# aapdo/M3ViT

Hardware: AMD Instinct MI355X
Metric: images/sec fwd+bwd ViT-S/16 MoE(E=16,k=4) 224^2 bs=128 (higher is better)
Workload: dtype f16; 1 GPU; configs[1]: ViT-Small/16 + MoE E=16 top-k=4 multi_gate, synthetic 224x224; batch_per_gpu=128, global_batch=128, task_passes=2, launch=hipGraph replay (one linear graph per task pass and stream), routing=deterministic (std=0), task_streams=2, wgrad_streams=0, activation_checkpointing=False, parallelism=single, full=False

## Files before the change

### m3vit_amd/csrc/gemm.hip

```cpp
#include <stdlib.h>
#include "gemm_dev.h"

using namespace m3;

struct GemmEnv {
  int band;
  bool dma;
  bool tall;
};
static int env_int(const char *name, int unset) { const char *e = getenv(name); return e ? atoi(e) : unset; }
static const GemmEnv &gemm_env() {
  static const GemmEnv env = {env_int("M3_GEMM_BAND", 0), env_int("M3_GEMM_DMA", 1) != 0, env_int("M3_GEMM_F32_TALL", 1) != 0};
  return env;
}

static int g_big_mode = -1;
extern "C" int m3_gemm_set_big(int mode) {
  M3_REQUIRE(mode >= -1 && mode <= 2, "m3_gemm_set_big: mode %d out of range", mode);
  g_big_mode = mode;
  return M3_OK;
}

static int epilogue_kind(const m3_gemm_args *a) {
  if (dtype_size(a->dtype) != 2) return DMA_EPI_ANY;
  const bool c_f32 = a->c_dtype == M3_F32, none = a->act == M3_ACT_NONE && !a->pre_out;
  if (none && a->gelu_grad_pre && !a->residual && !c_f32 && !a->bias) return DMA_EPI_GPRE;
  if (none && a->residual && !a->gelu_grad_pre && c_f32) return DMA_EPI_RES;
  if (none && !a->gelu_grad_pre && !a->residual && !c_f32) return DMA_EPI_PLAIN;
  if (a->act == M3_ACT_GELU && a->pre_out && !a->gelu_grad_pre && !a->residual && !c_f32) return DMA_EPI_GELU;
  return DMA_EPI_ANY;
}

enum GemmKernel { GEMM_BIG, GEMM_DMA, GEMM_STAGED, GEMM_STAGED_TALL };

static GemmKernel choose_kernel(const GemmDev &d, int dtype) {
  const GemmEnv &env = gemm_env();
  const int es = dtype_size(dtype);
  if (g_big_mode < 0) g_big_mode = env_int("M3_GEMM_BIG", 2);
  if (g_big_mode && gemm_big_eligible(d, es, g_big_mode == 1)) return GEMM_BIG;
  if (env.dma && es == 2 && d.vec8 && (d.K * es) % ROWB == 0) return GEMM_DMA;
  if (env.tall && dtype == M3_F32 && (d.K * es) % ROWB == 0 && !d.group_offsets) {
    const int64_t nt = (d.N + BN - 1) / BN, t128 = (d.M + 127) / 128 * nt, t160 = (d.M + 159) / 160 * nt;
    if ((t160 + 255) / 256 * 160 < (t128 + 255) / 256 * 128) return GEMM_STAGED_TALL;
  }
  return GEMM_STAGED;
}

struct GemmLaunch { GemmDev d; GemmKernel kernel; int epi, tile_m, tile_n; bool empty; };
static int gemm_prepare(const m3_gemm_args *a, const char *who, GemmLaunch &L) {
  M3_REQUIRE(a && a->A && a->B && a->C, "%s: null operand", who);
  M3_REQUIRE(dtype_ok(a->dtype), "%s: bad dtype %d", who, a->dtype);
  const int es = dtype_size(a->dtype);
  M3_REQUIRE(a->M >= 0 && a->N > 0 && a->K > 0, "%s: bad shape M=%lld N=%d K=%d", who, (long long)a->M, a->N, a->K);
  M3_REQUIRE((a->K * es) % 16 == 0, "%s: K*elem (%d) must be a multiple of 16 bytes", who, a->K * es);
  M3_REQUIRE((a->lda * es) % 16 == 0 && (a->ldb * es) % 16 == 0, "%s: lda/ldb rows must be 16-byte aligned", who);
  M3_REQUIRE(((uintptr_t)a->A % 16) == 0 && ((uintptr_t)a->B % 16) == 0 && ((uintptr_t)a->C % 16) == 0,
             "%s: operands must be 16-byte aligned", who);
  M3_REQUIRE(a->N % 4 == 0 && a->ldc % 4 == 0, "%s: N and ldc must be multiples of 4", who);
  M3_REQUIRE(a->lda >= a->K && a->ldb >= a->K && a->ldc >= a->N, "%s: leading dimension too small", who);
  M3_REQUIRE(a->c_dtype == M3_F32 || a->c_dtype == a->dtype, "%s: c_dtype must be f32 or the operand dtype", who);
  M3_REQUIRE(a->G >= 1, "%s: G must be >= 1", who);
  M3_REQUIRE((a->group_offsets == nullptr) == (a->tile_starts == nullptr), "%s: group_offsets/tile_starts go together", who);
  M3_REQUIRE(a->G == 1 || a->group_offsets, "%s: grouped call needs group_offsets", who);
  M3_REQUIRE(!a->a_row_idx || a->a_row_div >= 1, "%s: a_row_div must be >= 1", who);
  M3_REQUIRE(!a->pre_out || a->ld_pre % 4 == 0, "%s: ld_pre %% 4", who);
  M3_REQUIRE(!a->gelu_grad_pre || a->ld_gpre % 4 == 0, "%s: ld_gpre %% 4", who);
  M3_REQUIRE(!a->residual || a->ld_res % 4 == 0, "%s: ld_res %% 4", who);
  M3_REQUIRE(!a->row_scale || a->row_scale_div >= 1, "%s: row_scale_div must be >= 1", who);
  L.empty = a->M == 0;
  if (L.empty) return M3_OK;

  GemmDev &d = L.d;
  d.A = (const char *)a->A; d.lda_b = a->lda * es;
  d.a_row_idx = a->a_row_idx; d.a_row_div = a->a_row_idx ? a->a_row_div : 1;
  d.a_row_sh = div_shift(d.a_row_div);
  d.B = (const char *)a->B; d.ldb_b = a->ldb * es; d.b_group_b = (int64_t)a->N * a->ldb * es;
  d.C = (char *)a->C; d.ldc = a->ldc; d.c_f32 = (a->c_dtype == M3_F32) ? 1 : 0;
  d.c_row_idx = a->c_row_idx;
  d.bias = a->bias;
  d.pre_out = (char *)a->pre_out; d.ld_pre = a->ld_pre;
  d.gpre = (const char *)a->gelu_grad_pre; d.ld_gpre = a->ld_gpre;
  d.residual = a->residual; d.ld_res = a->ld_res;
  d.row_scale = a->row_scale; d.row_scale_div = a->row_scale ? a->row_scale_div : 1;
  d.row_scale_idx = a->row_scale ? a->row_scale_idx : nullptr;
  d.act = a->act;
  d.M = a->M; d.N = a->N; d.K = a->K; d.G = a->G;
  d.group_offsets = a->group_offsets; d.tile_starts = a->tile_starts;
  d.a_seg_tiles = 0; d.a_seg_jump_b = 0;
  d.vec8 = (a->N % 8 == 0 && a->ldc % 8 == 0 && (!a->pre_out || a->ld_pre % 8 == 0) &&
            (!a->gelu_grad_pre || a->ld_gpre % 8 == 0) && (!a->residual || a->ld_res % 8 == 0)) ? 1 : 0;
  M3_REQUIRE((a->M + 1) * a->lda * es < ((int64_t)1 << 32) && (int64_t)a->N * a->ldb * es < ((int64_t)1 << 32),
             "%s: operand panel exceeds the 4 GiB reach of the 32-bit lane offsets", who);

  const GemmKernel kernel = L.kernel = choose_kernel(d, a->dtype);
  L.epi = kernel == GEMM_BIG || kernel == GEMM_DMA ? epilogue_kind(a) : DMA_EPI_ANY;
  const int tile_m = L.tile_m = kernel == GEMM_BIG ? BIG_B : kernel == GEMM_STAGED_TALL ? 160 : BM;
  const int tile_n = L.tile_n = kernel == GEMM_BIG ? BIG_B : BN;
  const int band = gemm_env().band > 0 ? gemm_env().band : ((int64_t)a->N * a->K * es > ((int64_t)2 << 20) ? 4 : 1);
  const int64_t mt = (a->M + tile_m - 1) / tile_m + (a->group_offsets ? a->G : 0);
  d.n_tiles = (a->N + tile_n - 1) / tile_n;
  d.m_band = kernel == GEMM_BIG ? 1 : band;
  M3_REQUIRE(mt * d.n_tiles < (int64_t)1 << 30, "%s: grid too large", who);
  d.m_tiles_max = (int)mt;
  return M3_OK;
}

extern "C" int m3_gemm_nt(const m3_gemm_args *a, void *stream) {
  GemmLaunch L;
  if (int rc = gemm_prepare(a, "m3_gemm_nt", L)) return rc;
  if (L.empty) return M3_OK;
  hipStream_t s = (hipStream_t)stream;
  switch (L.kernel) {
    case GEMM_BIG: return launch_gemm_big(L.d, a->dtype, L.epi, s);
    case GEMM_DMA: return launch_gemm_dma(L.d, a->dtype, L.epi, s);
    default: return launch_gemm_staged(L.d, a->dtype, L.kernel == GEMM_STAGED_TALL, s);
  }
}

extern "C" int m3_gemm_plan(const m3_gemm_args *a, m3_gemm_plan_out *p) {
  M3_REQUIRE(p, "m3_gemm_plan: null output");
  GemmLaunch L;
  if (int rc = gemm_prepare(a, "m3_gemm_plan", L)) return rc;
  *p = m3_gemm_plan_out{};
  p->kernel = M3_GEMM_NONE;
  if (L.empty) return M3_OK;
  p->kernel = L.kernel == GEMM_BIG ? M3_GEMM_BIG : L.kernel == GEMM_DMA ? M3_GEMM_DMA : L.kernel == GEMM_STAGED_TALL ? M3_GEMM_STAGED_TALL : M3_GEMM_STAGED;
  p->epilogue = L.epi; p->tile_m = L.tile_m; p->tile_n = L.tile_n; p->m_band = L.d.m_band; p->vec8 = L.d.vec8;
  p->n_tiles = L.d.n_tiles; p->m_tiles_max = L.d.m_tiles_max;
  return M3_OK;
}
```

### m3vit_amd/csrc/gemm_dev.h

```cpp
#pragma once
#include <type_traits>
#include "common.h"

namespace m3 {

constexpr int BM = 128, BN = 128, ROWB = 128;
constexpr int GEMM_THREADS = 256;

struct GemmDev {
  const char *A; int64_t lda_b;
  const int32_t *a_row_idx; int32_t a_row_div; int32_t a_row_sh;
  const char *B; int64_t ldb_b; int64_t b_group_b;
  char *C; int64_t ldc; int32_t c_f32;
  const int32_t *c_row_idx;
  const float *bias;
  char *pre_out; int64_t ld_pre;
  const char *gpre; int64_t ld_gpre;
  const float *residual; int64_t ld_res;
  const float *row_scale; int32_t row_scale_div;
  const int32_t *row_scale_idx;
  int32_t act;
  int64_t M; int32_t N; int32_t K;
  int32_t G;
  const int32_t *group_offsets;
  const int32_t *tile_starts;
  int32_t n_tiles;
  int32_t m_band;
  int32_t m_tiles_max;
  int32_t vec8;
  int32_t a_seg_tiles; int64_t a_seg_jump_b;
};

struct TileOwner { int g; int64_t m_begin, m_end; };
__device__ __forceinline__ int grouped_live_tiles(const int32_t *tile_starts, int G, int lane, int &ts_lane) {
  if (G <= 64) {
    ts_lane = lane < G ? tile_starts[lane + 1] : 0x7fffffff;
    return __builtin_amdgcn_readfirstlane(__shfl(ts_lane, G - 1, 64));
  }
  ts_lane = 0;
  return tile_starts[G];
}
template <int ROWS>
__device__ __forceinline__ TileOwner grouped_tile_rows(const int32_t *group_offsets, int g, int t0, int mt) {
  TileOwner o;
  g = __builtin_amdgcn_readfirstlane(g);
  t0 = __builtin_amdgcn_readfirstlane(t0);
  o.g = g;
  o.m_begin = (int64_t)__builtin_amdgcn_readfirstlane(group_offsets[g]) + (int64_t)(mt - t0) * ROWS;
  o.m_end = __builtin_amdgcn_readfirstlane(group_offsets[g + 1]);
  return o;
}
__device__ __forceinline__ TileOwner grouped_tile_owner(const int32_t *tile_starts, const int32_t *group_offsets, int G,
                                                        int mt, int lane, int ts_lane) {
  int g = 0, t0;
  if (G <= 64) {
    g = __popcll(__ballot(lane < G - 1 && ts_lane <= mt));
    t0 = g ? __shfl(ts_lane, g - 1, 64) : 0;
  } else {
    while (g + 1 < G && tile_starts[g + 1] <= mt) ++g;
    t0 = tile_starts[g];
  }
  return grouped_tile_rows<128>(group_offsets, g, t0, mt);
}

__device__ __forceinline__ int dma_swz(int row) { return (row >> 1) & 7; }

enum { DMA_EPI_ANY = 0, DMA_EPI_GPRE = 1, DMA_EPI_RES = 2, DMA_EPI_PLAIN = 3, DMA_EPI_GELU = 4 };

template <typename F> inline void with_epi(int epi, F &&f) {
  switch (epi) {
    case DMA_EPI_GPRE: f(std::integral_constant<int, DMA_EPI_GPRE>()); break;
    case DMA_EPI_RES: f(std::integral_constant<int, DMA_EPI_RES>()); break;
    case DMA_EPI_PLAIN: f(std::integral_constant<int, DMA_EPI_PLAIN>()); break;
    case DMA_EPI_GELU: f(std::integral_constant<int, DMA_EPI_GELU>()); break;
    default: f(std::integral_constant<int, DMA_EPI_ANY>()); break;
  }
}

template <typename T, typename RowFactor>
__device__ __forceinline__ void epilogue_row_any(const GemmDev &p, int64_t m, int n, f32x4 v0, f32x4 v1, RowFactor row_factor) {
  const int64_t crow = p.c_row_idx ? (int64_t)p.c_row_idx[m] : m;
  if (p.pre_out) Vec8<T>::store((T *)p.pre_out + crow * p.ld_pre + n, v0, v1);
  if (p.act == M3_ACT_GELU) {
#pragma unroll
    for (int j = 0; j < 4; ++j) { v0[j] = gelu_f(v0[j]); v1[j] = gelu_f(v1[j]); }
  }
  if (p.gpre) {
    f32x4 p0, p1;
    Vec8<T>::load((const T *)p.gpre + crow * p.ld_gpre + n, p0, p1);
#pragma unroll
    for (int j = 0; j < 4; ++j) { v0[j] *= gelu_grad_f(p0[j]); v1[j] *= gelu_grad_f(p1[j]); }
  }
  if (p.row_scale) {
    const float sc = row_factor(crow);
    v0 *= sc; v1 *= sc;
  }
  if (p.residual) {
    v0 += *(const f32x4 *)(p.residual + crow * p.ld_res + n);
    v1 += *(const f32x4 *)(p.residual + crow * p.ld_res + n + 4);
  }
  if (p.c_f32) {
    *(f32x4 *)((float *)p.C + crow * p.ldc + n) = v0;
    *(f32x4 *)((float *)p.C + crow * p.ldc + n + 4) = v1;
  } else {
    Vec8<T>::store((T *)p.C + crow * p.ldc + n, v0, v1);
  }
}

constexpr int BIG_B = 256;
int launch_gemm_staged(const GemmDev &d, int dtype, bool tall, hipStream_t s);
int launch_gemm_dma(const GemmDev &d, int dtype, int epi, hipStream_t s);
bool gemm_big_eligible(const GemmDev &d, int dtype_size_bytes, bool force);
int launch_gemm_big(const GemmDev &d, int dtype, int epi, hipStream_t s);
int launch_gemm_big_seg(const GemmDev &d, int dtype, hipStream_t s, const char *who);

__device__ __forceinline__ void tile_of(int t, int n_tiles, int m_band, int live_m, int &mt, int &nt) {
  if (m_band <= 1) { mt = t / n_tiles; nt = t - mt * n_tiles; return; }
  const int per = m_band * n_tiles;
  const int band = t / per, r = t - band * per;
  const int rows = min(m_band, live_m - band * m_band);
  nt = r / rows;
  mt = band * m_band + (r - nt * rows);
}
}
```

### m3vit_amd/csrc/gemm_dma.hip

```cpp
#include "gemm_dev.h"

namespace m3 {

constexpr int DMA_RB = 128;
constexpr int DMA_LDS = 2 * BM * DMA_RB;
constexpr int DMA_LDS_ALL = DMA_LDS + BM * 4;

template <typename T, int EPI, bool HINT>
__global__ __launch_bounds__(GEMM_THREADS, 4) void gemm_nt_dma_kernel(const GemmDev p) {
  typedef Mma<T> MM;
  typedef typename MM::frag frag;
  constexpr int RB = DMA_RB;
  constexpr int OPB = BM * RB;
  constexpr int CPR = RB / 16;
  constexpr int RPI = 64 / CPR;
  constexpr int NPC = BM / RPI / 4;
  constexpr int KCH = RB / 64;
  extern __shared__ __attribute__((aligned(16))) char smem[];

  const int tid = threadIdx.x;
  const int lane = tid & 63, wave = __builtin_amdgcn_readfirstlane(tid >> 6);
  const int li = lane & 15, lg = lane >> 4;
  const int wr = wave >> 1, wc = wave & 1;

  int ts_lane = 0;
  const int nwg = p.tile_starts ? grouped_live_tiles(p.tile_starts, p.G, lane, ts_lane) * p.n_tiles : (int)gridDim.x;
  if ((int)blockIdx.x >= nwg) return;
  const int t = xcd_remap(blockIdx.x, nwg);
  int mt, nt;
  tile_of(t, p.n_tiles, p.m_band, nwg / p.n_tiles, mt, nt);
  int g = 0;
  int64_t m_begin, m_end;
  if (p.tile_starts) {
    const TileOwner ow = grouped_tile_owner(p.tile_starts, p.group_offsets, p.G, mt, lane, ts_lane);
    g = ow.g; m_begin = ow.m_begin; m_end = ow.m_end;
  } else {
    m_begin = (int64_t)mt * BM;
    m_end = p.M;
    if (m_begin >= m_end) return;
  }
  const int n0 = nt * BN;

  const char *a_src[NPC], *b_src[NPC];
  int64_t mrow[NPC];
  int32_t aix[NPC];
#pragma unroll
  for (int j = 0; j < NPC; ++j) {
    const int row = (NPC * wave + j) * RPI + lane / CPR;
    int64_t m = m_begin + row;
    if (m >= m_end) m = m_end - 1;
    mrow[j] = m;
  }
  if (p.a_row_idx) {
#pragma unroll
    for (int j = 0; j < NPC; ++j) aix[j] = p.a_row_idx[mrow[j]];
  }
  const bool want_rs = p.row_scale && tid < BM;
  const int32_t *rs_idx = p.row_scale_idx ? p.row_scale_idx : p.c_row_idx;
  int64_t rs_m = m_begin + tid;
  if (rs_m >= m_end) rs_m = m_end - 1;
  int32_t rs_ix = 0;
  if (want_rs && rs_idx) rs_ix = rs_idx[rs_m];
  float my_rs = 1.0f;
  if (want_rs) {
    const int64_t srow = rs_idx ? (int64_t)rs_ix : rs_m;
    my_rs = p.row_scale[p.row_scale_div == 1 ? srow : srow / p.row_scale_div];
  }
#pragma unroll
  for (int j = 0; j < NPC; ++j) {
    const int row = (NPC * wave + j) * RPI + lane / CPR;
    const int c = (lane % CPR) ^ dma_swz(row);
    const int64_t src = p.a_row_idx ? (int64_t)div_by(aix[j], p.a_row_div, p.a_row_sh) : mrow[j];
    a_src[j] = p.A + src * p.lda_b + c * 16;
    int n = n0 + row;
    if (n >= p.N) n = p.N - 1;
    b_src[j] = p.B + (int64_t)g * p.b_group_b + (int64_t)n * p.ldb_b + c * 16;
  }
  const int nk = (p.K * (int)sizeof(T)) / RB;

  typedef __attribute__((address_space(3))) void lds_void;
  typedef const __attribute__((address_space(1))) void glb_void;
  auto dma = [&](int ks) {
    char *dst = smem + (NPC * wave) * 1024;
#pragma unroll
    for (int j = 0; j < NPC; ++j) {
      __builtin_amdgcn_global_load_lds((glb_void *)(a_src[j] + ks * RB), (lds_void *)(dst + j * 1024), 16, 0, 0);
      __builtin_amdgcn_global_load_lds((glb_void *)(b_src[j] + ks * RB), (lds_void *)(dst + j * 1024 + OPB), 16, 0, 0);
    }
  };

  int rdA[KCH], rdB[KCH];
#pragma unroll
  for (int kc = 0; kc < KCH; ++kc) {
    rdA[kc] = (wr * 64 + li) * RB + (((kc * 4 + lg) ^ dma_swz(li)) << 4);
    rdB[kc] = (wc * 64 + li) * RB + (((kc * 4 + lg) ^ dma_swz(li)) << 4) + OPB;
  }

  f32x4 acc[4][4];
#pragma unroll
  for (int a = 0; a < 4; ++a)
#pragma unroll
    for (int b = 0; b < 4; ++b) acc[a][b] = f32x4{0.f, 0.f, 0.f, 0.f};

  auto compute = [&]() {
    const char *sb = smem;
#pragma unroll
    for (int kc = 0; kc < KCH; ++kc) {
      frag fa[4], fb[4];
#pragma unroll
      for (int i = 0; i < 4; ++i) {
        fa[i] = *(const frag *)(sb + rdA[kc] + i * 16 * RB);
        fb[i] = *(const frag *)(sb + rdB[kc] + i * 16 * RB);
      }
#pragma unroll
      for (int ni = 0; ni < 4; ++ni)
#pragma unroll
        for (int mi = 0; mi < 4; ++mi) acc[ni][mi] = MM::mma(fb[ni], fa[mi], acc[ni][mi]);
    }
  };

  for (int ks = 0; ks < nk; ++ks) {
    dma(ks);
    __syncthreads();
    compute();
    __syncthreads();
  }

  const float *bias = p.bias ? p.bias + (int64_t)g * p.N : nullptr;
  const int cg = tid & 15, r16 = tid >> 4;
  const int n = n0 + cg * 8;
  f32x4 b0 = f32x4{0.f, 0.f, 0.f, 0.f}, b1 = b0;
  if (bias && n < p.N) { b0 = *(const f32x4 *)(bias + n); b1 = *(const f32x4 *)(bias + n + 4); }
  float *const s_rs = (float *)(smem + DMA_LDS);
  if (tid < BM) s_rs[tid] = my_rs;
#pragma unroll
  for (int h = 0; h < 2; ++h) {
    u32x4 gq[4];
    f32x4 rq[4][2];
    int32_t crow4[4];
    constexpr int NPRE = EPI == DMA_EPI_RES ? 2 : 4;
    auto fetch_epi = [&](int ps) {
      if constexpr (EPI == DMA_EPI_GPRE) gq[ps] = ld_nt<HINT>((const u32x4 *)((const T *)p.gpre + (int64_t)crow4[ps] * p.ld_gpre + n));
      if constexpr (EPI == DMA_EPI_RES) {
        rq[ps][0] = *(const f32x4 *)(p.residual + (int64_t)crow4[ps] * p.ld_res + n);
        rq[ps][1] = *(const f32x4 *)(p.residual + (int64_t)crow4[ps] * p.ld_res + n + 4);
      }
    };
    if constexpr (EPI != DMA_EPI_ANY) {
      if (n < p.N) {
#pragma unroll
        for (int ps = 0; ps < 4; ++ps) {
          int64_t m = m_begin + h * 64 + ps * 16 + r16;
          if (m >= m_end) m = m_end - 1;
          crow4[ps] = p.c_row_idx ? p.c_row_idx[m] : (int32_t)m;
        }
#pragma unroll
        for (int ps = 0; ps < NPRE; ++ps) fetch_epi(ps);
      }
    }
    if (h) __syncthreads();
    if (wr == h) {
#pragma unroll
      for (int mi = 0; mi < 4; ++mi)
#pragma unroll
        for (int ni = 0; ni < 4; ++ni) {
          const int lrow = mi * 16 + li;
          const int chunk = wc * 16 + ni * 4 + lg;
          *(f32x4 *)(smem + lrow * 512 + ((chunk ^ (lrow & 31)) << 4)) = acc[ni][mi];
        }
    }
    __syncthreads();
    if constexpr (EPI != DMA_EPI_ANY) {
      if (n < p.N) {
#pragma unroll
        for (int ps = NPRE; ps < 4; ++ps) fetch_epi(ps);
#pragma unroll
        for (int ps = 0; ps < 4; ++ps) {
          const int lrow = ps * 16 + r16;
          const int64_t crow = crow4[ps];
          const int sw = lrow & 31;
          f32x4 v0 = *(const f32x4 *)(smem + lrow * 512 + (((2 * cg) ^ sw) << 4));
          f32x4 v1 = *(const f32x4 *)(smem + lrow * 512 + (((2 * cg + 1) ^ sw) << 4));
          v0 += b0; v1 += b1;
          if constexpr (EPI == DMA_EPI_GELU) {
            if constexpr (HINT) st_nt<true>((u32x4 *)((T *)p.pre_out + crow * p.ld_pre + n), pack8<T>(v0, v1));
            else Vec8<T>::store((T *)p.pre_out + crow * p.ld_pre + n, v0, v1);
#pragma unroll
            for (int j = 0; j < 4; ++j) { v0[j] = gelu_f(v0[j]); v1[j] = gelu_f(v1[j]); }
          }
          if constexpr (EPI == DMA_EPI_GPRE) {
            typedef T t8 __attribute__((ext_vector_type(8)));
            const t8 pr = __builtin_bit_cast(t8, gq[ps]);
#pragma unroll
            for (int j = 0; j < 4; ++j) { v0[j] *= gelu_grad_f((float)pr[j]); v1[j] *= gelu_grad_f((float)pr[4 + j]); }
          }
          const float sc = s_rs[h * 64 + lrow];
          v0 *= sc; v1 *= sc;
          if constexpr (EPI == DMA_EPI_RES) {
            v0 += rq[ps][0]; v1 += rq[ps][1];
            if (m_begin + h * 64 + lrow < m_end) {
              *(f32x4 *)((float *)p.C + crow * p.ldc + n) = v0;
              *(f32x4 *)((float *)p.C + crow * p.ldc + n + 4) = v1;
            }
          } else {
            Vec8<T>::store((T *)p.C + crow * p.ldc + n, v0, v1);
          }
        }
      }
    } else if (n < p.N) {
#pragma unroll 2
      for (int ps = 0; ps < 4; ++ps) {
        const int lrow = ps * 16 + r16;
        const int64_t m = m_begin + h * 64 + lrow;
        if (m >= m_end) break;
        const int sw = lrow & 31;
        const f32x4 v0 = *(const f32x4 *)(smem + lrow * 512 + (((2 * cg) ^ sw) << 4));
        const f32x4 v1 = *(const f32x4 *)(smem + lrow * 512 + (((2 * cg + 1) ^ sw) << 4));
        epilogue_row_any<T>(p, m, n, v0 + b0, v1 + b1, [&](int64_t) { return s_rs[h * 64 + lrow]; });
      }
    }
  }
}

int launch_gemm_dma(const GemmDev &d, int dtype, int epi, hipStream_t s) {
  const dim3 grid((unsigned)((int64_t)d.m_tiles_max * d.n_tiles)), block(GEMM_THREADS);
  const int hints = cache_hints();
  auto go = [&](auto t) {
    with_epi(epi, [&](auto e) {
      constexpr int EPI = decltype(e)::value;
      constexpr int BIT = EPI == DMA_EPI_GELU ? M3_HINT_GEMM_PRE : EPI == DMA_EPI_GPRE ? M3_HINT_GEMM_GPRE : 0;
      if (BIT && (hints & BIT)) {
        hipLaunchKernelGGL((gemm_nt_dma_kernel<decltype(t), EPI, BIT != 0>), grid, block, DMA_LDS_ALL, s, d);
      } else {
        hipLaunchKernelGGL((gemm_nt_dma_kernel<decltype(t), EPI, false>), grid, block, DMA_LDS_ALL, s, d);
      }
    });
  };
  if (dtype == M3_F16) go(half_t());
  else go(bf16_t());
  return check_launch("m3_gemm_nt");
}

}
```

Before: 8002 images/s.

## Shrink DMA GEMM prologue: scalar params, 32-bit offsets, hoisted first load

The DMA GEMM kernel now copies its parameters into values pinned to scalar registers. It replaces 64-bit per-piece source pointers with 32-bit lane offsets from a scalar base, and computes tile row bounds in 32-bit arithmetic with a precomputed shift for row-scale division. The first K-slice DMA is issued before the loop, and each later slice is issued after the compute barrier. This shortens the prologue and cuts VGPR pressure. A new host check limits M to 32 bits, and optional timestamp instrumentation is added behind a compile flag.

```diff
diff --git a/m3vit_amd/csrc/gemm.hip b/m3vit_amd/csrc/gemm.hip
--- a/m3vit_amd/csrc/gemm.hip
+++ b/m3vit_amd/csrc/gemm.hip
@@ -83,6 +83,7 @@
   d.residual = a->residual; d.ld_res = a->ld_res;
   d.row_scale = a->row_scale; d.row_scale_div = a->row_scale ? a->row_scale_div : 1;
   d.row_scale_idx = a->row_scale ? a->row_scale_idx : nullptr;
+  d.row_scale_sh = div_shift(d.row_scale_div);
   d.act = a->act;
   d.M = a->M; d.N = a->N; d.K = a->K; d.G = a->G;
   d.group_offsets = a->group_offsets; d.tile_starts = a->tile_starts;
@@ -91,6 +92,7 @@
             (!a->gelu_grad_pre || a->ld_gpre % 8 == 0) && (!a->residual || a->ld_res % 8 == 0)) ? 1 : 0;
   M3_REQUIRE((a->M + 1) * a->lda * es < ((int64_t)1 << 32) && (int64_t)a->N * a->ldb * es < ((int64_t)1 << 32),
              "%s: operand panel exceeds the 4 GiB reach of the 32-bit lane offsets", who);
+  M3_REQUIRE(a->M < ((int64_t)1 << 31), "%s: M %lld does not fit 32 bits", who, (long long)a->M);
 
   const GemmKernel kernel = L.kernel = choose_kernel(d, a->dtype);
   L.epi = kernel == GEMM_BIG || kernel == GEMM_DMA ? epilogue_kind(a) : DMA_EPI_ANY;
diff --git a/m3vit_amd/csrc/gemm_dev.h b/m3vit_amd/csrc/gemm_dev.h
--- a/m3vit_amd/csrc/gemm_dev.h
+++ b/m3vit_amd/csrc/gemm_dev.h
@@ -19,6 +19,7 @@
   const float *residual; int64_t ld_res;
   const float *row_scale; int32_t row_scale_div;
   const int32_t *row_scale_idx;
+  int32_t row_scale_sh;
   int32_t act;
   int64_t M; int32_t N; int32_t K;
   int32_t G;
@@ -50,9 +51,9 @@
   o.m_end = __builtin_amdgcn_readfirstlane(group_offsets[g + 1]);
   return o;
 }
-__device__ __forceinline__ TileOwner grouped_tile_owner(const int32_t *tile_starts, const int32_t *group_offsets, int G,
-                                                        int mt, int lane, int ts_lane) {
-  int g = 0, t0;
+__device__ __forceinline__ void grouped_tile_group(const int32_t *tile_starts, int G, int mt, int lane, int ts_lane, int &g,
+                                                   int &t0) {
+  g = 0;
   if (G <= 64) {
     g = __popcll(__ballot(lane < G - 1 && ts_lane <= mt));
     t0 = g ? __shfl(ts_lane, g - 1, 64) : 0;
@@ -60,6 +61,11 @@
     while (g + 1 < G && tile_starts[g + 1] <= mt) ++g;
     t0 = tile_starts[g];
   }
+}
+__device__ __forceinline__ TileOwner grouped_tile_owner(const int32_t *tile_starts, const int32_t *group_offsets, int G,
+                                                        int mt, int lane, int ts_lane) {
+  int g, t0;
+  grouped_tile_group(tile_starts, G, mt, lane, ts_lane, g, t0);
   return grouped_tile_rows<128>(group_offsets, g, t0, mt);
 }
 
diff --git a/m3vit_amd/csrc/gemm_dma.hip b/m3vit_amd/csrc/gemm_dma.hip
--- a/m3vit_amd/csrc/gemm_dma.hip
+++ b/m3vit_amd/csrc/gemm_dma.hip
@@ -5,6 +5,17 @@
 constexpr int DMA_RB = 128;
 constexpr int DMA_LDS = 2 * BM * DMA_RB;
 constexpr int DMA_LDS_ALL = DMA_LDS + BM * 4;
+
+#ifdef M3_GEMM_STAMPS
+constexpr int STAMP_WGS = 4096, STAMP_N = 64;
+__device__ unsigned long long g_gemm_stamps[STAMP_WGS][STAMP_N];
+#define M3_GEMM_STAMP(i)                                                                                              \
+  do {                                                                                                                \
+    if (threadIdx.x == 0 && blockIdx.x < STAMP_WGS && (i) < STAMP_N) g_gemm_stamps[blockIdx.x][(i)] = __builtin_amdgcn_s_memtime(); \
+  } while (0)
+#else
+#define M3_GEMM_STAMP(i) do { } while (0)
+#endif
 
 template <typename T, int EPI, bool HINT>
 __global__ __launch_bounds__(GEMM_THREADS, 4) void gemm_nt_dma_kernel(const GemmDev p) {
@@ -18,76 +29,120 @@
   constexpr int KCH = RB / 64;
   extern __shared__ __attribute__((aligned(16))) char smem[];
 
+  M3_GEMM_STAMP(0);
+  const char *const A = p.A, *const B = p.B;
+  const int64_t lda_b = p.lda_b, ldb_b = p.ldb_b, b_group_b = p.b_group_b, M = p.M;
+  const int32_t *const a_row_idx = p.a_row_idx, *const c_row_idx = p.c_row_idx, *const row_scale_idx = p.row_scale_idx;
+  const int32_t *const group_offsets = p.group_offsets, *const tile_starts = p.tile_starts;
+  const float *const row_scale = p.row_scale;
+  const int a_row_div = p.a_row_div, a_row_sh = p.a_row_sh, row_scale_div = p.row_scale_div, row_scale_sh = p.row_scale_sh;
+  const int N = p.N, K = p.K, G = p.G, n_tiles = p.n_tiles, m_band = p.m_band, m_tiles_max = p.m_tiles_max;
+  asm volatile("" ::"s"(A), "s"(B), "s"(lda_b), "s"(ldb_b), "s"(b_group_b), "s"(M), "s"(a_row_idx), "s"(c_row_idx),
+               "s"(row_scale_idx), "s"(group_offsets), "s"(tile_starts), "s"(row_scale), "s"(a_row_div), "s"(a_row_sh),
+               "s"(row_scale_div), "s"(row_scale_sh), "s"(N), "s"(K), "s"(G), "s"(n_tiles), "s"(m_band), "s"(m_tiles_max));
+
   const int tid = threadIdx.x;
   const int lane = tid & 63, wave = __builtin_amdgcn_readfirstlane(tid >> 6);
   const int li = lane & 15, lg = lane >> 4;
   const int wr = wave >> 1, wc = wave & 1;
 
   int ts_lane = 0;
-  const int nwg = p.tile_starts ? grouped_live_tiles(p.tile_starts, p.G, lane, ts_lane) * p.n_tiles : (int)gridDim.x;
+  const int live_m = tile_starts ? grouped_live_tiles(tile_starts, G, lane, ts_lane) : m_tiles_max;
+  const int nwg = live_m * n_tiles;
   if ((int)blockIdx.x >= nwg) return;
   const int t = xcd_remap(blockIdx.x, nwg);
   int mt, nt;
-  tile_of(t, p.n_tiles, p.m_band, nwg / p.n_tiles, mt, nt);
-  int g = 0;
-  int64_t m_begin, m_end;
-  if (p.tile_starts) {
-    const TileOwner ow = grouped_tile_owner(p.tile_starts, p.group_offsets, p.G, mt, lane, ts_lane);
-    g = ow.g; m_begin = ow.m_begin; m_end = ow.m_end;
-  } else {
-    m_begin = (int64_t)mt * BM;
-    m_end = p.M;
-    if (m_begin >= m_end) return;
+  tile_of(t, n_tiles, m_band, live_m, mt, nt);
+  int g = 0, t0 = 0, go_begin = 0, go_end = 0;
+  if (tile_starts) {
+    typedef const __attribute__((address_space(4))) int32_t const_i32;
+    grouped_tile_group(tile_starts, G, mt, lane, ts_lane, g, t0);
+    g = __builtin_amdgcn_readfirstlane(g);
+    t0 = __builtin_amdgcn_readfirstlane(t0);
+    go_begin = ((const_i32 *)group_offsets)[g];
+    go_end = ((const_i32 *)group_offsets)[g + 1];
+  } else if ((int64_t)mt * BM >= M) {
+    return;
   }
   const int n0 = nt * BN;
-
-  const char *a_src[NPC], *b_src[NPC];
-  int64_t mrow[NPC];
-  int32_t aix[NPC];
-#pragma unroll
-  for (int j = 0; j < NPC; ++j) {
-    const int row = (NPC * wave + j) * RPI + lane / CPR;
-    int64_t m = m_begin + row;
-    if (m >= m_end) m = m_end - 1;
-    mrow[j] = m;
-  }
-  if (p.a_row_idx) {
-#pragma unroll
-    for (int j = 0; j < NPC; ++j) aix[j] = p.a_row_idx[mrow[j]];
-  }
-  const bool want_rs = p.row_scale && tid < BM;
-  const int32_t *rs_idx = p.row_scale_idx ? p.row_scale_idx : p.c_row_idx;
-  int64_t rs_m = m_begin + tid;
-  if (rs_m >= m_end) rs_m = m_end - 1;
-  int32_t rs_ix = 0;
-  if (want_rs && rs_idx) rs_ix = rs_idx[rs_m];
-  float my_rs = 1.0f;
-  if (want_rs) {
-    const int64_t srow = rs_idx ? (int64_t)rs_ix : rs_m;
-    my_rs = p.row_scale[p.row_scale_div == 1 ? srow : srow / p.row_scale_div];
-  }
+  const int nk = (K * (int)sizeof(T)) / RB;
+
+  typedef __attribute__((address_space(3))) void lds_void;
+  typedef const __attribute__((address_space(1))) void glb_void;
+  uint32_t a_off[NPC], b_off[NPC];
+  const char *const Bg = B + (int64_t)g * b_group_b;
+  char *const dma_dst = smem + (NPC * wave) * 1024;
+  auto dma_b = [&](int ks) {
+    const char *base = Bg + ks * RB;
+    asm("" : "+s"(base));
+#pragma unroll
+    for (int j = 0; j < NPC; ++j) {
+      uint32_t off = b_off[j];
+      asm volatile("" : "+v"(off));
+      __builtin_amdgcn_global_load_lds((glb_void *)(base + off), (lds_void *)(dma_dst + j * 1024 + OPB), 16, 0, 0);
+    }
+  };
+  auto dma_a = [&](int ks) {
+    const char *base = A + ks * RB;
+    asm("" : "+s"(base));
+#pragma unroll
+    for (int j = 0; j < NPC; ++j) {
+      uint32_t off = a_off[j];
+      asm volatile("" : "+v"(off));
+      __builtin_amdgcn_global_load_lds((glb_void *)(base + off), (lds_void *)(dma_dst + j * 1024), 16, 0, 0);
+    }
+  };
+
 #pragma unroll
   for (int j = 0; j < NPC; ++j) {
     const int row = (NPC * wave + j) * RPI + lane / CPR;
     const int c = (lane % CPR) ^ dma_swz(row);
-    const int64_t src = p.a_row_idx ? (int64_t)div_by(aix[j], p.a_row_div, p.a_row_sh) : mrow[j];
-    a_src[j] = p.A + src * p.lda_b + c * 16;
     int n = n0 + row;
-    if (n >= p.N) n = p.N - 1;
-    b_src[j] = p.B + (int64_t)g * p.b_group_b + (int64_t)n * p.ldb_b + c * 16;
-  }
-  const int nk = (p.K * (int)sizeof(T)) / RB;
-
-  typedef __attribute__((address_space(3))) void lds_void;
-  typedef const __attribute__((address_space(1))) void glb_void;
-  auto dma = [&](int ks) {
-    char *dst = smem + (NPC * wave) * 1024;
-#pragma unroll
-    for (int j = 0; j < NPC; ++j) {
-      __builtin_amdgcn_global_load_lds((glb_void *)(a_src[j] + ks * RB), (lds_void *)(dst + j * 1024), 16, 0, 0);
-      __builtin_amdgcn_global_load_lds((glb_void *)(b_src[j] + ks * RB), (lds_void *)(dst + j * 1024 + OPB), 16, 0, 0);
-    }
-  };
+    if (n >= N) n = N - 1;
+    b_off[j] = (uint32_t)n * (uint32_t)ldb_b + c * 16;
+  }
+
+  const int mb32 = tile_starts ? go_begin + (mt - t0) * BM : mt * BM;
+  const int me32 = tile_starts ? go_end : (int)M;
+  int32_t mrow[NPC], aix[NPC];
+#pragma unroll
+  for (int j = 0; j < NPC; ++j) {
+    int m = mb32 + (NPC * wave + j) * RPI + lane / CPR;
+    if (m >= me32) m = me32 - 1;
+    mrow[j] = m;
+  }
+  const bool want_rs = row_scale && tid < BM;
+  const int32_t *const rs_idx = row_scale_idx ? row_scale_idx : c_row_idx;
+  int rs_m = mb32 + tid;
+  if (rs_m >= me32) rs_m = me32 - 1;
+  int32_t rs_ix = rs_m;
+  if (a_row_idx) {
+#pragma unroll
+    for (int j = 0; j < NPC; ++j) aix[j] = a_row_idx[mrow[j]];
+  }
+  if (want_rs && rs_idx) rs_ix = rs_idx[rs_m];
+  if (a_row_idx) {
+    if (a_row_sh >= 0) {
+#pragma unroll
+      for (int j = 0; j < NPC; ++j) mrow[j] = aix[j] >> a_row_sh;
+    } else {
+#pragma unroll
+      for (int j = 0; j < NPC; ++j) mrow[j] = aix[j] / a_row_div;
+    }
+  }
+#pragma unroll
+  for (int j = 0; j < NPC; ++j) {
+    const int row = (NPC * wave + j) * RPI + lane / CPR;
+    const int c = (lane % CPR) ^ dma_swz(row);
+    a_off[j] = (uint32_t)mrow[j] * (uint32_t)lda_b + c * 16;
+  }
+  asm volatile("" : "+v"(a_off[0]), "+v"(a_off[1]), "+v"(a_off[2]), "+v"(a_off[3]));
+  static_assert(NPC == 4, "the pin above names four pieces");
+  float my_rs = 1.0f;
+  if (want_rs) my_rs = row_scale[div_by(rs_ix, row_scale_div, row_scale_sh)];
+  M3_GEMM_STAMP(1);
+  dma_b(0);
+  dma_a(0);
 
   int rdA[KCH], rdB[KCH];
 #pragma unroll
@@ -119,11 +174,15 @@
     }
   };
 
-  for (int ks = 0; ks < nk; ++ks) {
-    dma(ks);
+  for (int ks = 0;;) {
     __syncthreads();
+    if (ks < 27) M3_GEMM_STAMP(2 + 2 * ks);
     compute();
     __syncthreads();
+    if (ks < 27) M3_GEMM_STAMP(3 + 2 * ks);
+    if (++ks >= nk) break;
+    dma_a(ks);
+    dma_b(ks);
   }
 
   const float *bias = p.bias ? p.bias + (int64_t)g * p.N : nullptr;
@@ -150,9 +209,9 @@
       if (n < p.N) {
 #pragma unroll
         for (int ps = 0; ps < 4; ++ps) {
-          int64_t m = m_begin + h * 64 + ps * 16 + r16;
-          if (m >= m_end) m = m_end - 1;
-          crow4[ps] = p.c_row_idx ? p.c_row_idx[m] : (int32_t)m;
+          int m = mb32 + h * 64 + ps * 16 + r16;
+          if (m >= me32) m = me32 - 1;
+          crow4[ps] = c_row_idx ? c_row_idx[m] : m;
         }
 #pragma unroll
         for (int ps = 0; ps < NPRE; ++ps) fetch_epi(ps);
@@ -160,12 +219,14 @@
     }
     if (h) __syncthreads();
     if (wr == h) {
+      int sli = li, slg = lg;
+      asm volatile("" : "+v"(sli), "+v"(slg));
 #pragma unroll
       for (int mi = 0; mi < 4; ++mi)
 #pragma unroll
         for (int ni = 0; ni < 4; ++ni) {
-          const int lrow = mi * 16 + li;
-          const int chunk = wc * 16 + ni * 4 + lg;
+          const int lrow = mi * 16 + sli;
+          const int chunk = wc * 16 + ni * 4 + slg;
           *(f32x4 *)(smem + lrow * 512 + ((chunk ^ (lrow & 31)) << 4)) = acc[ni][mi];
         }
     }
@@ -198,7 +259,7 @@
           v0 *= sc; v1 *= sc;
           if constexpr (EPI == DMA_EPI_RES) {
             v0 += rq[ps][0]; v1 += rq[ps][1];
-            if (m_begin + h * 64 + lrow < m_end) {
+            if (mb32 + h * 64 + lrow < me32) {
               *(f32x4 *)((float *)p.C + crow * p.ldc + n) = v0;
               *(f32x4 *)((float *)p.C + crow * p.ldc + n + 4) = v1;
             }
@@ -211,15 +272,20 @@
 #pragma unroll 2
       for (int ps = 0; ps < 4; ++ps) {
         const int lrow = ps * 16 + r16;
-        const int64_t m = m_begin + h * 64 + lrow;
-        if (m >= m_end) break;
+        const int m = mb32 + h * 64 + lrow;
+        if (m >= me32) break;
         const int sw = lrow & 31;
         const f32x4 v0 = *(const f32x4 *)(smem + lrow * 512 + (((2 * cg) ^ sw) << 4));
         const f32x4 v1 = *(const f32x4 *)(smem + lrow * 512 + (((2 * cg + 1) ^ sw) << 4));
         epilogue_row_any<T>(p, m, n, v0 + b0, v1 + b1, [&](int64_t) { return s_rs[h * 64 + lrow]; });
       }
     }
-  }
+    M3_GEMM_STAMP(56 + h);
+  }
+#ifdef M3_GEMM_STAMPS
+  asm volatile("s_waitcnt vmcnt(0)" ::: "memory");
+  M3_GEMM_STAMP(58);
+#endif
 }
 
 int launch_gemm_dma(const GemmDev &d, int dtype, int epi, hipStream_t s) {
@@ -242,3 +308,17 @@
 }
 
 }
+
+#ifdef M3_GEMM_STAMPS
+extern "C" int m3_debug_gemm_stamps(unsigned long long *dst, int wgs, int clear) {
+  using namespace m3;
+  if (wgs > STAMP_WGS) wgs = STAMP_WGS;
+  const size_t bytes = (size_t)wgs * STAMP_N * sizeof(unsigned long long);
+  if (dst && hipMemcpyFromSymbol(dst, HIP_SYMBOL(g_gemm_stamps), bytes) != hipSuccess) return M3_ERR_LAUNCH;
+  if (clear) {
+    void *sym = nullptr;
+    if (hipGetSymbolAddress(&sym, HIP_SYMBOL(g_gemm_stamps)) != hipSuccess || hipMemset(sym, 0, sizeof(g_gemm_stamps)) != hipSuccess) return M3_ERR_LAUNCH;
+  }
+  return M3_OK;
+}
+#endif
```

Result: faster. 8120 images/s, median of 6 (+1.5%).
